# atenpas/gpd

Measured on NVIDIA H100. Metric: grasp candidates/sec end-to-end (15ch), higher is better.
Workload: dtype f64 geometry / f32 LeNet

## Files before the change

### gpd_b200/csrc/api.cu

```cuda
#include <atomic>
#include <cfloat>
#include <cmath>
#include <cstdarg>
#include <cstdio>
#include <cstdlib>
#include <cstring>
#include <initializer_list>
#include <string>
#include <utility>
#include <vector>

#include "../../include/gpd_b200_depth.h"
#include "../../include/gpd_b200_outliers.h"
#include "../../include/gpd_b200_plane.h"
#include "../../include/gpd_b200_refine.h"
#include "common.cuh"

static char g_create_err[512] = "";

struct StageTimes {
  struct Span { int stage; cudaEvent_t b, e; };
  std::vector<cudaEvent_t> pool;
  size_t used = 0;
  std::vector<Span> spans;
// ... 2560 lines not shown
    return GPDB_ERR_STATE;
  }
  const SisState &st = *ctx->sis;
  const int B = st.B, R = st.R, S = st.S, RS = R * S;
  SisArena a;
  carve_at(ctx->scratch[SCR_SIS], [&](Carve &c) { sis_layout(c, B, R, S, st.init_off[B], a); });
  CUDA_TRY(cudaSetDevice(ctx->device));
  std::vector<double> ev(eval_xyz_out ? 3 * (size_t)B * RS : 0), kp(kept_xyz_out ? 3 * ((size_t)st.init_off[B] + (size_t)B * RS) : 0);
  if (!ev.empty()) CUDA_TRY(cudaMemcpyAsync(ev.data(), a.eval, sizeof(double) * ev.size(), cudaMemcpyDeviceToHost, ctx->stream));
  if (!kp.empty()) CUDA_TRY(cudaMemcpyAsync(kp.data(), a.kept, sizeof(double) * kp.size(), cudaMemcpyDeviceToHost, ctx->stream));
  CUDA_TRY(cudaStreamSynchronize(ctx->stream));
  if (eval_offsets_out || eval_round_counts_out || eval_xyz_out) {
    size_t o = 0;
    if (eval_offsets_out) eval_offsets_out[0] = 0;
    for (int b = 0; b < B; b++) {
      for (int r = 0; r < R; r++) {
        const int c = st.ecount[(size_t)r * B + b];
        if (eval_round_counts_out) eval_round_counts_out[(size_t)b * R + r] = c;
        if (eval_xyz_out) memcpy(eval_xyz_out + 3 * o, ev.data() + 3 * ((size_t)b * R + r) * S, sizeof(double) * 3 * c);
        o += c;
      }
      if (eval_offsets_out) eval_offsets_out[b + 1] = (int32_t)o;
    }
  }
  if (kept_offsets_out) memcpy(kept_offsets_out, st.koff.data(), sizeof(int32_t) * ((size_t)B + 1));
  if (kept_xyz_out)
    for (int b = 0; b < B; b++)
      memcpy(kept_xyz_out + 3 * (size_t)st.koff[b], kp.data() + 3 * ((size_t)st.init_off[b] + (size_t)b * RS),
             sizeof(double) * 3 * (size_t)(st.koff[b + 1] - st.koff[b]));
  return B;
}

void gpdb_free_result(gpdb_result *r) {
  if (!r) return;
  if (r->owner_) {
    HostArena *a = (HostArena *)r->owner_;
    a->in_use = false;
    arena_unref(a);
  } else {
    free(r->frame_valid);
    free(r->frames);
    free(r->pose_flags);
    free(r->pose_scores);
    free(r->candidates);
    free(r->images);
  }
  memset(r, 0, sizeof(*r));
}

int gpdb_debug_phase_cycles(gpdb_ctx *ctx, int enable, uint64_t cycles_out[32]) {
  if (!ctx) return GPDB_ERR_INVALID;
  CUDA_TRY(cudaSetDevice(ctx->device));
  CUDA_TRY(cudaStreamSynchronize(ctx->stream));
  if (ctx->d_prof && cycles_out) {
    CUDA_TRY(cudaMemcpy(cycles_out, ctx->d_prof, sizeof(uint64_t) * 16, cudaMemcpyDeviceToHost));
    CUDA_TRY(cudaMemcpy(cycles_out + 16, ctx->d_prof + GPDB_PROF_SUB, sizeof(uint64_t) * 16, cudaMemcpyDeviceToHost));
  }
  if (enable && !ctx->d_prof) CUDA_TRY(cudaMalloc(&ctx->d_prof, sizeof(uint64_t) * GPDB_PROF_SLOTS));
  if (enable) CUDA_TRY(cudaMemset(ctx->d_prof, 0, sizeof(uint64_t) * GPDB_PROF_SLOTS));
  if (!enable && ctx->d_prof) {
    cudaFree(ctx->d_prof);
    ctx->d_prof = nullptr;
  }
  return GPDB_OK;
}

int gpdb_debug_path_counts(gpdb_ctx *ctx, uint64_t counts_out[16]) {
  if (!ctx || !counts_out) return GPDB_ERR_INVALID;
  CUDA_TRY(cudaSetDevice(ctx->device));
  CUDA_TRY(cudaStreamSynchronize(ctx->stream));
  if (ctx->d_prof)
    CUDA_TRY(cudaMemcpy(counts_out, ctx->d_prof + GPDB_PROF_PATH, sizeof(uint64_t) * 16, cudaMemcpyDeviceToHost));
  else
    memset(counts_out, 0, sizeof(uint64_t) * 16);
  return GPDB_OK;
}

int gpdb_last_timings(const gpdb_ctx *ctx, double ms_out[8]) {
  if (!ctx || !ms_out) return GPDB_ERR_INVALID;
  for (int i = 0; i < 8; i++) ms_out[i] = ctx->last_ms[i];
  return GPDB_OK;
}

}
```

### gpd_b200/csrc/common.cuh

```cuda
#pragma once
#include <cuda_runtime.h>
#include <stdint.h>

#include "../../include/gpd_b200.h"
#include "../../include/gpd_b200_shadow.h"

#define GPDB_MAX_ORIENT 32
#define GPDB_MAX_SLOTS 32
#define GPDB_MAX_DEEPEN 64
#define GPDB_MAX_NSP 128

struct DevParams {
  double finger_width, hand_outer_diameter, hand_depth, hand_height, init_bite;
  int P, n_axes, n_orient, nfp;
  int axes[GPDB_MAX_HAND_AXES];
  int deepen, slots_disjoint, all_axes_z;
  double inv_slot_step;
  double fs[GPDB_MAX_SLOTS];
  double fsw[GPDB_MAX_SLOTS];
  int J;
  double topj[GPDB_MAX_DEEPEN], botj[GPDB_MAX_DEEPEN];
  double cosf;
  int min_viable;
  double min_ap, max_ap, ws[6];
// ... 23 lines not shown
  const float *xyz;
  const double *nrm;
  const uint8_t *cam;
  const int *cell_start;
  const double *samples;
  int n_points;
};

struct CloudDesc {
  float lo[3], inv_cell;
  int dim[3];
  int cell_base;
  int off, N, K;
  int all_seen;
  int nonunit;
  int pos;
  double vp[GPDB_MAX_CAMERAS][3];
};
struct CloudTable {
  const CloudDesc *d;
  const int *soff;
  int n;
};

struct CloudSet {
  float4 *pts4;
  float *xyz;
  double *nrm;
  uint8_t *cam;
  int *src;
  int *cell_start;
  CloudDesc *desc;
  int *soff;
  int *off;
  int *sel;
  int *pos;
  int *raw_off;
  size_t point_cap, cell_cap, desc_cap;
  int n, maxk;
  bool has_src;
  double *samples;
  int n_samples;
  size_t samples_cap;
  int positions(int b) const { return n_samples ? pos[b + 1] - pos[b] : 0; }
  DevCloud view;
  int points() const { return n ? off[n] : 0; }
  CloudTable table() const { return CloudTable{desc, soff, n}; }
};

#define GPDB_NERR 8

#define GPDB_PROF_PATH 16
#define GPDB_PROF_SUB 32
#define GPDB_PROF_SLOTS 48
enum PathEvent {
  PATH_FRAMES_T1, PATH_FRAMES_T2, PATH_HANDS_T2, PATH_HANDS_T3, PATH_HANDS_SLAB, PATH_IMG2_BOX, PATH_IMG2_NONUNIT, PATH_IMG_GL,
  PATH_IMG2_CAST, PATH_IMG2_DRAW, PATH_IMG2_STASH, PATH_IMG_CAST, PATH_IMG_DRAW, PATH_IMG_STASH, PATH_IMG_BALL, PATH_LABEL_WALK
};

#define CUDA_TRY(expr)                                                                        \
  do {                                                                                        \
    cudaError_t e__ = (expr);                                                                 \
    if (e__ != cudaSuccess) {                                                                 \
      gpdb_set_error(ctx, GPDB_ERR_CUDA, "%s:%d %s -> %s", __FILE__, __LINE__, #expr,         \
                     cudaGetErrorString(e__));                                                \
      return GPDB_ERR_CUDA;                                                                   \
    }                                                                                         \
  } while (0)

#define LAUNCH_CHECK()                                                                                    \
  do {                                                                                                    \
    ctx->launches++;                                                                                      \
    cudaError_t e__ = cudaGetLastError();                                                                 \
    if (e__ != cudaSuccess) {                                                                             \
      gpdb_set_error(ctx, GPDB_ERR_CUDA, "%s:%d launch -> %s", __FILE__, __LINE__, cudaGetErrorString(e__)); \
      return GPDB_ERR_CUDA;                                                                               \
    }                                                                                                     \
  } while (0)

struct LenetWeights {
  float *c1w, *c1b, *c2w, *c2b, *i1w, *i1b, *i2w, *i2b;
  int C;
  bool set;
};

struct C1Affine {
  float scale[20], bias[20];
};
struct LenetTc {
  void *b1, *b2, *b3;
  C1Affine c1_aff;
  int npl, nch1;
  float w2_scale, a2_scale, w3_scale, x3_scale;
  bool ready;
};

struct StageTimes;
struct PipeState;
struct CommState;
struct SisState;

enum ScratchSlot {
  SCR_P16,
  SCR_CUB,
  SCR_OVF,
  SCR_KEYS,
  SCR_WORK_A, SCR_WORK_B, SCR_WORK_C,
// ... 240 lines not shown
```

### gpd_b200/csrc/geometry.cu

```cuda
#include <cfloat>
#include <climits>
#include <cstdlib>
#include <vector>
#include <cub/cub.cuh>

#include "common.cuh"
#include "grid.cuh"

namespace {

constexpr int NT_HANDS = 256;
#ifndef GPDB_NT_IMG
#define GPDB_NT_IMG 512
#endif
constexpr int NT_IMG = GPDB_NT_IMG;
constexpr int LRF_WARPS = 4;
constexpr int LRF_CAP_GLOBAL = 16384;
constexpr int LRF_CAP = 1024;
constexpr int BOX_CAP = 2048;
constexpr int MAXPIX = 64 * 64;

__device__ __forceinline__ void to_frame(const double *F, double v0, double v1, double v2, double &o0, double &o1,
                                         double &o2) {
  o0 = (F[0] * v0 + F[1] * v1) + F[2] * v2;
  o1 = (F[3] * v0 + F[4] * v1) + F[5] * v2;
  o2 = (F[6] * v0 + F[7] * v1) + F[8] * v2;
}
__device__ __forceinline__ void mat3_mul(const double *A, const double *B, double *Cm) {
#pragma unroll
  for (int c = 0; c < 3; c++)
#pragma unroll
    for (int r = 0; r < 3; r++) Cm[c * 3 + r] = (A[r] * B[c * 3] + A[3 + r] * B[c * 3 + 1]) + A[6 + r] * B[c * 3 + 2];
}

__device__ __forceinline__ double warp_min(double v) {
#pragma unroll
  for (int o = 16; o; o >>= 1) v = fmin(v, __shfl_xor_sync(0xffffffffu, v, o));
  return v;
}
__device__ __forceinline__ double warp_max(double v) {
#pragma unroll
  for (int o = 16; o; o >>= 1) v = fmax(v, __shfl_xor_sync(0xffffffffu, v, o));
  return v;
}
__device__ __forceinline__ int warp_sum(int v) { return __reduce_add_sync(0xffffffffu, v); }

template <int NT>
struct SegScan {
  typedef cub::BlockScan<int, NT> Scan;
  typename Scan::TempStorage tmp;
  int start[NT];
  int prefix[NT + 1];
};
template <int NT, class G>
__device__ __forceinline__ int seg_batch(const G &P, const int *cell_start, const SegRange &s, int row0,
                                         SegScan<NT> &seg) {
  int row = row0 + threadIdx.x, st = 0, len = 0;
  if (row < s.nrows) seg_row(P, cell_start, s, row, st, len);
  int excl, total;
  SegScan<NT>::Scan(seg.tmp).ExclusiveSum(len, excl, total);
  seg.start[threadIdx.x] = st;
  seg.prefix[threadIdx.x] = excl;
  if (threadIdx.x == 0) seg.prefix[NT] = total;
  __syncthreads();
  return total;
}
template <int NT, class G, class F>
__device__ __forceinline__ void scan_balanced(const G &P, const DevCloud &cl, const SegRange &sr, SegScan<NT> &seg,
                                              F &&body) {
  const int warp = threadIdx.x >> 5, lane = threadIdx.x & 31;
  constexpr int NW = NT / 32;
  for (int row0 = 0; row0 < sr.nrows; row0 += NT) {
    __syncthreads();
    const int total = seg_batch<NT>(P, cl.cell_start, sr, row0, seg);
    const int nr = min(NT, sr.nrows - row0);
    const int c_begin = (int)(((long long)total * warp) / NW), c_end = (int)(((long long)total * (warp + 1)) / NW);
    if (c_begin >= c_end) continue;
    int lo = 0, hi = nr;
    while (hi - lo > 1) {
      int mid = (lo + hi) >> 1;
      if (seg.prefix[mid] <= c_begin) lo = mid; else hi = mid;
    }
    int r = lo, c = c_begin;
    auto fetch = [&](bool &have, bool &in, float4 &p, int &where) {
      have = false;
      in = false;
      where = 0;
      p = make_float4(0.f, 0.f, 0.f, 0.f);
      while (c < c_end) {
        const int pe = (r + 1 < nr) ? seg.prefix[r + 1] : total;
        const int seg_end = min(pe, c_end);
        if (c >= seg_end) {
          r++;
          continue;
        }
        const int k = c + lane;
        in = k < seg_end;
        where = (seg.start[r] - seg.prefix[r]) + k;
        if (in) p = __ldg(cl.pts4 + where);
        c = min(c + 32, seg_end);
        have = true;
        return;
      }
    };
    bool have0, in0, have1, in1;
    float4 p0, p1;
    int w0, w1;
    fetch(have0, in0, p0, w0);
    while (have0) {
      fetch(have1, in1, p1, w1);
      body(in0, p0, w0);
      have0 = have1;
      in0 = in1;
      p0 = p1;
      w0 = w1;
    }
  }
}

template <int NT>
__device__ __forceinline__ int seg_lookup(const SegScan<NT> &seg, int c) {
  int lo = 0, hi = NT;
  while (hi - lo > 1) {
    int mid = (lo + hi) >> 1;
    if (seg.prefix[mid] <= c) lo = mid; else hi = mid;
  }
  return seg.start[lo] + (c - seg.prefix[lo]);
}

__device__ void make_givens(double p, double q, double &c, double &s) {
  if (q == 0.0) {
    c = p < 0.0 ? -1.0 : 1.0;
    s = 0.0;
  } else if (p == 0.0) {
    c = 0.0;
    s = q < 0.0 ? 1.0 : -1.0;
  } else if (fabs(p) > fabs(q)) {
    double t = q / p;
    double u = sqrt(1.0 + t * t);
    if (p < 0.0) u = -u;
    c = 1.0 / u;
    s = -t * c;
  } else {
    double t = p / q;
    double u = sqrt(1.0 + t * t);
    if (q < 0.0) u = -u;
    s = -1.0 / u;
    c = -t * s;
  }
}
__device__ double eigen_hypot(double x, double y) {
  double ax = fabs(x), ay = fabs(y);
  double p = fmax(ax, ay);
  if (p == 0.0) return 0.0;
  double qp = fmin(ax, ay) / p;
  return p * sqrt(1.0 + qp * qp);
}
__device__ void eigen3(const double *Min, double *eval, double *Q) {
  double m00 = Min[0], m10 = Min[1], m20 = Min[2], m11 = Min[4], m21 = Min[5], m22 = Min[8];
  double scale = fmax(fmax(fmax(fabs(m00), fabs(m10)), fmax(fabs(m20), fabs(m11))), fmax(fabs(m21), fabs(m22)));
  if (scale == 0.0) scale = 1.0;
  m00 /= scale; m10 /= scale; m20 /= scale; m11 /= scale; m21 /= scale; m22 /= scale;
  double diag[3], sub[2];
  const double tol = DBL_MIN;
  diag[0] = m00;
  double v1norm2 = m20 * m20;
  if (v1norm2 <= tol) {
    diag[1] = m11;
// ... 188 lines not shown
    double eval[3], evec[9];
    eigen3(M, eval, evec);
    int mn = 0, mx = 0;
    for (int k = 1; k < 3; k++) {
      if (eval[k] < eval[mn]) mn = k;
      if (eval[k] > eval[mx]) mx = k;
    }
    double curv[3] = {evec[mn * 3], evec[mn * 3 + 1], evec[mn * 3 + 2]};
    double normal[3] = {evec[mx * 3], evec[mx * 3 + 1], evec[mx * 3 + 2]};
    double nrm = sqrt((a[6] * a[6] + a[7] * a[7]) + a[8] * a[8]);
    double avg[3] = {a[6] / nrm, a[7] / nrm, a[8] / nrm};
    if ((avg[0] * normal[0] + avg[1] * normal[1]) + avg[2] * normal[2] < 0) {
      normal[0] *= -1.0; normal[1] *= -1.0; normal[2] *= -1.0;
    }
    double *f = frames + 9 * (size_t)i;
    f[0] = normal[0]; f[1] = normal[1]; f[2] = normal[2];
    f[3] = curv[1] * normal[2] - curv[2] * normal[1];
    f[4] = curv[2] * normal[0] - curv[0] * normal[2];
    f[5] = curv[0] * normal[1] - curv[1] * normal[0];
    f[6] = curv[0]; f[7] = curv[1]; f[8] = curv[2];
    valid[i] = 1;
  }
  return true;
}

__device__ __forceinline__ unsigned slot_mask(const DevParams &P, const double *sfs, const double *sfsw, double y) {
  unsigned m = 0;
  const int F = 2 * P.nfp;
  if (P.slots_disjoint) {
#pragma unroll
    for (int half = 0; half < 2; half++) {
      const double *fs = sfs + half * P.nfp, *fsw = sfsw + half * P.nfp;
      const double tq = (y - fs[0]) * P.inv_slot_step;
      const double tf = floor(tq);
      if (tq - tf > 1e-9 && tf + 1.0 - tq > 1e-9) {
        const int i = (int)tf;
        if (i >= 0 && i < P.nfp && y > fs[i] && y < fsw[i]) m |= 1u << (half * P.nfp + i);
      } else {
        const int e = min(max((int)tf, 1), P.nfp - 2 > 1 ? P.nfp - 2 : 1);
#pragma unroll
        for (int d = -1; d <= 1; d++) {
          const int i = e + d;
          if (i >= 0 && i < P.nfp && y > fs[i] && y < fsw[i]) m |= 1u << (half * P.nfp + i);
        }
      }
    }
  } else {
    for (int f = 0; f < F; f++)
      if (y > sfs[f] && y < sfsw[f]) m |= 1u << f;
  }
  return m;
}

constexpr int SURV_CAP = 1024;
struct HandsSmem {
  SegScan<NT_HANDS> seg;
  unsigned short surv[NT_HANDS / 32][SURV_CAP];
  double fs[GPDB_MAX_SLOTS], fsw[GPDB_MAX_SLOTS];
  int count;
  int n_ball;
  unsigned long long nb0_key;
  double T[9];
  double frame[9];
  double sample[3];
  int cap;
};

template <bool BATCH>
__global__ void __launch_bounds__(NT_HANDS, 4) k_hands(const DevParams *Pp, DevCloud cl0, CloudTable tab, const int *sidx, int n, int slot0,
                                                    const double *frames, const uint8_t *fvalid, gpdb_pose *poses,
                                                    uint8_t *flags, int cap, const int *in_list, const int *in_count,
                                                    int *out_list, int *out_count, float4 *glist, int *err,
                                                    unsigned long long *prof) {
  const DevParams &P = *Pp;
  extern __shared__ __align__(16) unsigned char dyn[];
  float4 *list = glist ? glist + (size_t)blockIdx.x * cap : reinterpret_cast<float4 *>(dyn);
  __shared__ HandsSmem S;
  const int tid = threadIdx.x, lane = tid & 31, warp = tid >> 5;
  const int work_n = in_list ? *in_count : n;
  if (tid < 2 * P.nfp) {
    S.fs[tid] = P.fs[tid];
    S.fsw[tid] = P.fsw[tid];
  }
  for (int w = blockIdx.x; w < work_n; w += gridDim.x) {
    const int i = in_list ? in_list[w] : w;
    const int si = sidx[i];
    const auto &G = CloudSel<BATCH>::get(tab, slot0 + i);
    const DevCloud cl = CloudSel<BATCH>::local(G, cl0);
    __syncthreads();
    if (tid == 0) {
      S.count = 0;
      S.n_ball = 0;
      S.nb0_key = ~0ull;
    }
    if (tid < 9) S.frame[tid] = frames[9 * (size_t)i + tid];
    if (tid == 0) sample_position(cl, si, S.sample);
    __syncthreads();
    if (tid == 0) mat3_mul(S.frame, P.rotb, S.T);
    const bool fv = fvalid[i] != 0;
    if (!fv) {
      for (int p = tid; p < P.P; p += NT_HANDS) {
        gpdb_pose *h = poses + (size_t)i * P.P + p;
        memset(h, 0, sizeof(gpdb_pose));
        h->sample_index = si;
        h->sample_slot = slot0 + i;
        h->pose_slot = (int16_t)p;
        h->finger_idx = -1;
        h->score = __int_as_float(0x7fc00000);
        flags[(size_t)i * P.P + p] = 0;
      }
      continue;
    }
    __syncthreads();
    float q[3] = {(float)S.sample[0], (float)S.sample[1], (float)S.sample[2]};
    SegRange sr = seg_range(G, q, P.rf_hs);
    const double hz = P.hand_height * 1.001 + 1e-9;
    unsigned long long best = ~0ull;
    int nball = 0;
    scan_balanced<NT_HANDS>(G, cl, sr, S.seg, [&](bool in, const float4 &p, int) {
      bool keep = false;
      if (in) {
        float d = l2_simple(q, p.x, p.y, p.z);
        if (d < P.r2_hs) {
          nball++;
          unsigned long long key = ((unsigned long long)__float_as_uint(d) << 32) | (unsigned)__float_as_int(p.w);
          best = key < best ? key : best;
          keep = true;
          if (P.all_axes_z) {
            double z0 = (S.T[6] * ((double)p.x - S.sample[0]) + S.T[7] * ((double)p.y - S.sample[1])) +
                        S.T[8] * ((double)p.z - S.sample[2]);
            keep = fabs(z0) < hz;
          }
        }
      }
      unsigned m = __ballot_sync(0xffffffffu, keep);
      if (m) {
        int leader = __ffs(m) - 1, base = 0;
        if (lane == leader) base = atomicAdd(&S.count, __popc(m));
        base = __shfl_sync(0xffffffffu, base, leader);
        int pos = base + __popc(m & ((1u << lane) - 1));
        if (keep && pos < cap) list[pos] = p;
      }
    });
    nball = warp_sum(nball);
#pragma unroll
    for (int o = 16; o; o >>= 1) {
      unsigned long long ob = __shfl_xor_sync(0xffffffffu, best, o);
      best = ob < best ? ob : best;
    }
    if (lane == 0) {
      atomicAdd(&S.n_ball, nball);
      atomicMin(&S.nb0_key, best);
    }
    __syncthreads();
    const int m = S.count;
    if (m > cap) {
      if (tid == 0) {
        if (out_list) {
          int k = atomicAdd(out_count, 1);
          out_list[k] = i;
          if (!in_list) atomicAdd(err + 3, 1);
        } else {
          atomicAdd(err + 1, 1);
        }
      }
      if (!out_list) {
        for (int p = tid; p < P.P; p += NT_HANDS) flags[(size_t)i * P.P + p] = 0;
      }
      continue;
    }
    const int n_ball = S.n_ball;
    const int nb0 = (int)(unsigned)(S.nb0_key & 0xffffffffu);
    double nbx = 0, nby = 0, nbz = 0;
    if (n_ball > 0) {
      nbx = (double)cl.xyz[3 * (size_t)nb0] - S.sample[0];
      nby = (double)cl.xyz[3 * (size_t)nb0 + 1] - S.sample[1];
      nbz = (double)cl.xyz[3 * (size_t)nb0 + 2] - S.sample[2];
    }
    for (int pose = warp; pose < P.P; pose += NT_HANDS / 32) {
      gpdb_pose *h = poses + (size_t)i * P.P + pose;
      double R[9];
      mat3_mul(S.T, P.rot[pose], R);
      const double hh = P.hand_height;
      uint8_t fl = 0;
      double top = 0, bottom = 0, center = 0, width = 0;
      int fidx = -1, fpi = -1;
      bool half = false, full = false;
      double x0, y0, z0;
      to_frame(R, nbx, nby, nbz, x0, y0, z0);
      if (n_ball > 0) {
        const double b0 = P.init_bite, bot0 = P.init_bite - P.hand_depth;
        int k = 0;
        unsigned anyA = 0, anyB = 0, fmask = 0;
        for (int a = lane; a < m; a += 32) {
          float4 p = list[a];
          double x, y, z;
          to_frame(R, (double)p.x - S.sample[0], (double)p.y - S.sample[1], (double)p.z - S.sample[2], x, y, z);
          if (z > -1.0 * hh && z < hh) {
            k++;
            if (x < b0) {
              anyA = 1;
              if (x < bot0) anyB = 1;
              fmask |= slot_mask(P, S.fs, S.fsw, y);
            }
          }
        }
        k = warp_sum(k);
        const int npad = n_ball - k;
        if (npad > 0 && x0 < b0) {
          anyA = 1;
          if (x0 < bot0) anyB = 1;
          fmask |= slot_mask(P, S.fs, S.fsw, y0);
        }
        anyA = __reduce_or_sync(0xffffffffu, anyA);
        anyB = __reduce_or_sync(0xffffffffu, anyB);
        fmask = __reduce_or_sync(0xffffffffu, fmask);
        const unsigned allF = (2 * P.nfp >= 32) ? 0xffffffffu : ((1u << (2 * P.nfp)) - 1);
        unsigned freef = (anyA && !anyB) ? (~fmask & allF) : 0u;
        unsigned hand = freef & (freef >> P.nfp) & ((1u << P.nfp) - 1);
        if (hand) {
          int cntb = __popc(hand);
          int target = (cntb + 1) / 2;
          unsigned hm = hand;
          while (--target) hm &= hm - 1;
          fidx = __ffs(hm) - 1;
          fpi = P.deepen ? fidx : (__ffs(hand) - 1);
          top = b0;
          bottom = bot0;
          if (P.deepen) {
            int jf = P.J;
            const double sl0 = P.fs[fidx], sl1 = P.fsw[fidx], sr0 = P.fs[P.nfp + fidx], sr1 = P.fsw[P.nfp + fidx];
            const int J = P.J;
            auto visitB = [&](double x, double y) {
              if (J > 0 && x < P.botj[J - 1]) {
                int j = 0;
                while (!(x < P.botj[j])) j++;
                jf = min(jf, j);
              }
              if ((y > sl0 && y < sl1) || (y > sr0 && y < sr1)) {
                if (J > 0 && x < P.topj[J - 1]) {
                  int j = 0;
                  while (!(x < P.topj[j])) j++;
                  jf = min(jf, j);
                }
              }
            };
            for (int a = lane; a < m; a += 32) {
              float4 p = list[a];
              double x, y, z;
              to_frame(R, (double)p.x - S.sample[0], (double)p.y - S.sample[1], (double)p.z - S.sample[2], x, y, z);
              if (z > -1.0 * hh && z < hh) visitB(x, y);
            }
            if (npad > 0) visitB(x0, y0);
            jf = __reduce_min_sync(0xffffffffu, jf);
            if (jf > 0) {
              top = P.topj[jf - 1];
              bottom = P.botj[jf - 1];
            }
          }
          const double left = P.fsw[fidx], right = P.fs[P.nfp + fidx];
          center = 0.5 * (left + right);
          int cnt = 0;
          double mny = DBL_MAX, mxy = -DBL_MAX;
          unsigned short *surv = S.surv[warp];
          int nsurv = 0;
          for (int a0 = 0; a0 < m; a0 += 32) {
            const int a = a0 + lane;
            bool inr = false;
            if (a < m) {
              float4 p = list[a];
              double x, y, z;
              to_frame(R, (double)p.x - S.sample[0], (double)p.y - S.sample[1], (double)p.z - S.sample[2], x, y, z);
              if (z > -1.0 * hh && z < hh && x > bottom && x < top && y > left && y < right) {
                inr = true;
                cnt++;
                mny = fmin(mny, y);
                mxy = fmax(mxy, y);
              }
            }
            const unsigned mk = __ballot_sync(0xffffffffu, inr);
            const int pos = nsurv + __popc(mk & ((1u << lane) - 1));
            if (inr && pos < SURV_CAP) surv[pos] = (unsigned short)a;
            nsurv += __popc(mk);
          }
          const bool surv_ok = nsurv <= SURV_CAP && m <= 65535;
          __syncwarp();
          const bool nb_in = npad > 0 && x0 > bottom && x0 < top && y0 > left && y0 < right;
          cnt = warp_sum(cnt) + (nb_in ? npad : 0);
          mny = warp_min(mny);
          mxy = warp_max(mxy);
          if (nb_in) {
            mny = fmin(mny, y0);
            mxy = fmax(mxy, y0);
          }
          if (cnt > 0) {
            fl |= GPDB_POSE_VALID;
            width = mxy - mny;
            const double min_x = mny + 0.003, max_x = mxy - 0.003;
            int cl_ = 0, cr_ = 0;
            double lmaxx = -DBL_MAX, lminx = DBL_MAX, lmaxz = -DBL_MAX, lminz = DBL_MAX;
            double rmaxx = -DBL_MAX, rminx = DBL_MAX, rmaxz = -DBL_MAX, rminz = DBL_MAX;
            auto visitD = [&](double x, double y, double z, int idx, int wgt) {
              const double *nn = cl.nrm + 3 * (size_t)idx;
              double n0, n1, n2;
              to_frame(R, nn[0], nn[1], nn[2], n0, n1, n2);
              double ldot = (0.0 * n0 + -1.0 * n1) + 0.0 * n2;
              double rdot = (0.0 * n0 + 1.0 * n1) + 0.0 * n2;
              if (ldot > P.cosf && y < min_x) {
                cl_ += wgt;
                lmaxx = fmax(lmaxx, x); lminx = fmin(lminx, x); lmaxz = fmax(lmaxz, z); lminz = fmin(lminz, z);
              }
              if (rdot > P.cosf && y > max_x) {
                cr_ += wgt;
                rmaxx = fmax(rmaxx, x); rminx = fmin(rminx, x); rmaxz = fmax(rmaxz, z); rminz = fmin(rminz, z);
              }
            };
            if (surv_ok) {
              for (int sidx_ = lane; sidx_ < nsurv; sidx_ += 32) {
                float4 p = list[surv[sidx_]];
                double x, y, z;
                to_frame(R, (double)p.x - S.sample[0], (double)p.y - S.sample[1], (double)p.z - S.sample[2], x, y, z);
                visitD(x, y, z, __float_as_int(p.w), 1);
              }
            } else {
              if (prof && lane == 0) atomicAdd(prof + GPDB_PROF_PATH + PATH_HANDS_SLAB, 1ull);
              for (int a = lane; a < m; a += 32) {
                float4 p = list[a];
                double x, y, z;
                to_frame(R, (double)p.x - S.sample[0], (double)p.y - S.sample[1], (double)p.z - S.sample[2], x, y, z);
                if (z > -1.0 * hh && z < hh && x > bottom && x < top && y > left && y < right)
                  visitD(x, y, z, __float_as_int(p.w), 1);
              }
            }
            if (nb_in && lane == 0) visitD(x0, y0, z0, nb0, npad);
            cl_ = warp_sum(cl_);
            cr_ = warp_sum(cr_);
            half = cl_ > 0 || cr_ > 0;
            if (cl_ > 0 && cr_ > 0) {
              lmaxx = warp_max(lmaxx); lminx = warp_min(lminx); lmaxz = warp_max(lmaxz); lminz = warp_min(lminz);
              rmaxx = warp_max(rmaxx); rminx = warp_min(rminx); rmaxz = warp_max(rmaxz); rminz = warp_min(rminz);
              const double top_y = fmin(lmaxx, rmaxx), bot_y = fmax(lminx, rminx);
              const double top_z = fmin(lmaxz, rmaxz), bot_z = fmax(lminz, rminz);
              int nl = 0, nr = 0;
              auto visitE = [&](double x, double y, double z, int idx, int wgt) {
                const double *nn = cl.nrm + 3 * (size_t)idx;
                double n0, n1, n2;
                to_frame(R, nn[0], nn[1], nn[2], n0, n1, n2);
                double ldot = (0.0 * n0 + -1.0 * n1) + 0.0 * n2;
                double rdot = (0.0 * n0 + 1.0 * n1) + 0.0 * n2;
                bool inw = x >= bot_y && x <= top_y && z >= bot_z && z <= top_z;
                if (ldot > P.cosf && y < min_x && inw) nl += wgt;
                if (rdot > P.cosf && y > max_x && inw) nr += wgt;
              };
              if (surv_ok) {
                for (int sidx_ = lane; sidx_ < nsurv; sidx_ += 32) {
                  float4 p = list[surv[sidx_]];
                  double x, y, z;
                  to_frame(R, (double)p.x - S.sample[0], (double)p.y - S.sample[1], (double)p.z - S.sample[2], x, y, z);
                  visitE(x, y, z, __float_as_int(p.w), 1);
                }
              } else {
                for (int a = lane; a < m; a += 32) {
                  float4 p = list[a];
                  double x, y, z;
                  to_frame(R, (double)p.x - S.sample[0], (double)p.y - S.sample[1], (double)p.z - S.sample[2], x, y, z);
                  if (z > -1.0 * hh && z < hh && x > bottom && x < top && y > left && y < right)
                    visitE(x, y, z, __float_as_int(p.w), 1);
                }
              }
              if (nb_in && lane == 0) visitE(x0, y0, z0, nb0, npad);
              nl = warp_sum(nl);
              nr = warp_sum(nr);
              full = nl >= P.min_viable && nr >= P.min_viable;
            }
            if (half) fl |= GPDB_POSE_HALF;
            if (full) fl |= GPDB_POSE_FULL;
          }
        }
      }
      if (lane == 0) {
        gpdb_pose o;
        memset(&o, 0, sizeof(o));
        for (int r = 0; r < 3; r++) o.sample[r] = S.sample[r];
        for (int r = 0; r < 9; r++) o.frame[r] = R[r];
        o.sample_index = si;
        o.sample_slot = slot0 + i;
        o.pose_slot = (int16_t)pose;
        o.finger_idx = -1;
        o.score = __int_as_float(0x7fc00000);
        if (fl & GPDB_POSE_VALID) {
          o.top = top;
          o.bottom = bottom;
          o.center = center;
          o.width = width;
          o.finger_idx = (int16_t)fpi;
          o.half_antipodal = half;
          o.full_antipodal = full;
          for (int r = 0; r < 3; r++)
            o.position[r] = ((R[r] * bottom + R[3 + r] * center) + R[6 + r] * 0.0) + S.sample[r];
          const double half_width = 0.5 * P.hand_outer_diameter;
          bool ok = width >= P.min_ap && width <= P.max_ap;
          for (int r = 0; r < 3; r++) {
            double lb = o.position[r] + half_width * R[3 + r];
            double rb = o.position[r] - half_width * R[3 + r];
            double lt = lb + P.hand_depth * R[r];
            double rt = lb + P.hand_depth * R[r];
            double ap = o.position[r] - 0.05 * R[r];
            double mn = fmin(fmin(fmin(lb, rb), fmin(lt, rt)), ap);
            double mx = fmax(fmax(fmax(lb, rb), fmax(lt, rt)), ap);
            ok = ok && mn >= P.ws[2 * r] && mx <= P.ws[2 * r + 1];
          }
          if (ok && P.filt_dir) {
            double dot = (P.dir[0] * R[0] + P.dir[1] * R[1]) + P.dir[2] * R[2];
            if (dot >= -1.0 && dot <= 1.0 && dot < P.dir_keep) ok = false;
          }
          if (ok) fl |= GPDB_POSE_FILTERED;
        }
        *h = o;
        flags[(size_t)i * P.P + pose] = fl;
      }
    }
  }
}

__global__ void k_flag01(const uint8_t *flags, int n, int *f01) {
  int i = blockIdx.x * blockDim.x + threadIdx.x;
  if (i < n) f01[i] = (flags[i] & 3) == 3;
}
__global__ void k_scatter(const gpdb_pose *poses, const int *f01, const int *pos, int n, gpdb_pose *cand, int *count) {
  int i = blockIdx.x * blockDim.x + threadIdx.x;
  if (i >= n) return;
  if (f01[i]) cand[pos[i]] = poses[i];
  if (i == n - 1) *count = pos[i] + f01[i];
}
__global__ void k_scatter_scores(const gpdb_pose *cand, const float *scores, int nc, int slot0, int P, float *pose_scores,
                                 gpdb_pose *cand_out) {
  int i = blockIdx.x * blockDim.x + threadIdx.x;
  if (i >= nc) return;
  float s = scores[i];
  pose_scores[(size_t)(cand[i].sample_slot - slot0) * P + cand[i].pose_slot] = s;
  cand_out[i].score = s;
}

__global__ void k_select_keys(const gpdb_pose *cand, int n, unsigned *keys, int *vals) {
  int i = blockIdx.x * blockDim.x + threadIdx.x;
  if (i >= n) return;
  unsigned u = __float_as_uint(cand[i].score);
  u ^= (u >> 31) ? 0xFFFFFFFFu : 0x80000000u;
  keys[i] = ~u;
  vals[i] = i;
}
__global__ void k_gather_poses(const gpdb_pose *cand, const int *order, int k, gpdb_pose *out) {
  const int w = (blockIdx.x * blockDim.x + threadIdx.x) >> 5, lane = threadIdx.x & 31;
  if (w >= k) return;
  const int *src = reinterpret_cast<const int *>(cand + order[w]);
  int *dst = reinterpret_cast<int *>(out + w);
  for (int j = lane; j < (int)(sizeof(gpdb_pose) / 4); j += 32) dst[j] = src[j];
}

constexpr int LABEL_NT = 128;
constexpr int LABEL_CAP = 1024;

template <class F>
__device__ __forceinline__ void warp_scan_ball(const CloudDesc &G, const DevCloud &cl, const SegRange &sr, const float q[3], float r2,
                                               F &&body) {
  const int lane = threadIdx.x & 31;
  for (int j0 = 0; j0 < sr.nrows; j0 += 32) {
    const int myrow = j0 + lane;
    int st = 0, len = 0;
    if (myrow < sr.nrows) seg_row(G, cl.cell_start, sr, myrow, st, len);
    unsigned nonempty = __ballot_sync(0xffffffffu, len > 0);
    while (nonempty) {
      const int j = __ffs(nonempty) - 1;
// ... 1629 lines not shown
  if (!ctx->d_prof) return GPDB_OK;
  k_path_add<<<1, 1, 0, ctx->stream>>>(ctx->d_prof, e0, n0, e1, n1);
  CUDA_TRY(cudaGetLastError());
  return GPDB_OK;
}

static bool overflow_lists(gpdb_ctx *ctx, int n, int *&ovf, int *&ovf_count, int *&ovf2, int *&ovf2_count) {
  return gpdb_carve(ctx, SCR_OVF, [&](Carve &c) {
    ovf = c.take<int>(n); ovf_count = c.take<int>(1); ovf2 = c.take<int>(n); ovf2_count = c.take<int>(1);
  });
}

template <bool BATCH>
static int launch_frames(gpdb_ctx *ctx, const CloudSet &s, const int *d_sidx, int n, double *d_frames, uint8_t *d_valid) {
  const int cap0 = 128;
  const size_t smem0 = (size_t)2 * LRF_WARPS * cap0 * sizeof(unsigned long long);
  const size_t smem1 = (size_t)2 * LRF_WARPS * LRF_CAP * sizeof(unsigned long long);
  CUDA_TRY(cudaFuncSetAttribute(k_frames<BATCH>, cudaFuncAttributeMaxDynamicSharedMemorySize, (int)smem1));
  int *ovf, *ovf_count, *ovf2, *ovf2_count;
  if (!overflow_lists(ctx, n, ovf, ovf_count, ovf2, ovf2_count)) return GPDB_ERR_CUDA;
  const int g2 = 37;
  unsigned long long *gkeys =
      (unsigned long long *)gpdb_scratch(ctx, SCR_FRAMES_GL, sizeof(unsigned long long) * 2 * LRF_CAP_GLOBAL * (size_t)g2 * LRF_WARPS);
  if (!gkeys) return GPDB_ERR_CUDA;
  CUDA_TRY(cudaMemsetAsync(ovf_count, 0, sizeof(int), ctx->stream));
  CUDA_TRY(cudaMemsetAsync(ovf2_count, 0, sizeof(int), ctx->stream));
  const DevCloud &cl = s.view;
  const CloudTable tab = s.table();
  const int grid = (n + LRF_WARPS - 1) / LRF_WARPS;
  k_frames<BATCH><<<grid, LRF_WARPS * 32, smem0, ctx->stream>>>(ctx->dp, cl, tab, d_sidx, n, d_frames, d_valid, ctx->d_err, cap0,
                                                                ovf, ovf_count, ovf2, ovf2_count, nullptr, 0);
  LAUNCH_CHECK();
  k_frames<BATCH><<<grid, LRF_WARPS * 32, smem1, ctx->stream>>>(ctx->dp, cl, tab, d_sidx, n, d_frames, d_valid, ctx->d_err,
                                                                LRF_CAP, ovf, ovf_count, ovf2, ovf2_count, nullptr, 1);
  LAUNCH_CHECK();
  k_frames<BATCH><<<g2, LRF_WARPS * 32, 0, ctx->stream>>>(ctx->dp, cl, tab, d_sidx, n, d_frames, d_valid, ctx->d_err,
                                                          LRF_CAP_GLOBAL, ovf, ovf_count, ovf2, ovf2_count, gkeys, 2);
  LAUNCH_CHECK();
  return path_add(ctx, PATH_FRAMES_T1, ovf_count, PATH_FRAMES_T2, ovf2_count);
}

int geo_frames(gpdb_ctx *ctx, const CloudSet &s, const int *d_sidx, int n, double *d_frames, uint8_t *d_valid) {
  if (n <= 0) return GPDB_OK;
  return s.n > 1 ? launch_frames<true>(ctx, s, d_sidx, n, d_frames, d_valid)
                 : launch_frames<false>(ctx, s, d_sidx, n, d_frames, d_valid);
}

static const int HANDS_CAP1 = 2176, HANDS_CAP2 = 12800;
static const int HANDS_CAP3 = 131072;

template <bool BATCH>
static int launch_hands(gpdb_ctx *ctx, const CloudSet &s, const int *d_sidx, int n, int slot0, const double *d_frames,
                        const uint8_t *d_valid, gpdb_pose *d_poses, uint8_t *d_flags) {
  CUDA_TRY(cudaFuncSetAttribute(k_hands<BATCH>, cudaFuncAttributeMaxDynamicSharedMemorySize, HANDS_CAP2 * 16));
  int *ovf, *ovf_count, *ovf2, *ovf2_count;
  if (!overflow_lists(ctx, n, ovf, ovf_count, ovf2, ovf2_count)) return GPDB_ERR_CUDA;
  float4 *glist = (float4 *)gpdb_scratch(ctx, SCR_HANDS_GL, sizeof(float4) * (size_t)HANDS_CAP3 * ctx->sm_count);
  if (!glist) return GPDB_ERR_CUDA;
  CUDA_TRY(cudaMemsetAsync(ovf_count, 0, sizeof(int), ctx->stream));
  CUDA_TRY(cudaMemsetAsync(ovf2_count, 0, sizeof(int), ctx->stream));
  const DevCloud &cl = s.view;
  const CloudTable tab = s.table();
  k_hands<BATCH><<<n, NT_HANDS, HANDS_CAP1 * 16, ctx->stream>>>(ctx->dp, cl, tab, d_sidx, n, slot0, d_frames, d_valid, d_poses,
                                                                d_flags, HANDS_CAP1, nullptr, nullptr, ovf, ovf_count, nullptr,
                                                                ctx->d_err, ctx->d_prof);
  LAUNCH_CHECK();
  k_hands<BATCH><<<ctx->sm_count, NT_HANDS, HANDS_CAP2 * 16, ctx->stream>>>(ctx->dp, cl, tab, d_sidx, n, slot0, d_frames,
                                                                            d_valid, d_poses, d_flags, HANDS_CAP2, ovf,
                                                                            ovf_count, ovf2, ovf2_count, nullptr, ctx->d_err,
                                                                            ctx->d_prof);
  LAUNCH_CHECK();
  k_hands<BATCH><<<ctx->sm_count, NT_HANDS, 16, ctx->stream>>>(ctx->dp, cl, tab, d_sidx, n, slot0, d_frames, d_valid, d_poses,
                                                               d_flags, HANDS_CAP3, ovf2, ovf2_count, nullptr, nullptr, glist,
                                                               ctx->d_err, ctx->d_prof);
  LAUNCH_CHECK();
  return path_add(ctx, PATH_HANDS_T2, ovf_count, PATH_HANDS_T3, ovf2_count);
}

int geo_hands(gpdb_ctx *ctx, const CloudSet &s, const int *d_sidx, int n, int slot0, const double *d_frames,
              const uint8_t *d_valid, gpdb_pose *d_poses, uint8_t *d_flags) {
  if (n <= 0) return GPDB_OK;
  return s.n > 1 ? launch_hands<true>(ctx, s, d_sidx, n, slot0, d_frames, d_valid, d_poses, d_flags)
                 : launch_hands<false>(ctx, s, d_sidx, n, slot0, d_frames, d_valid, d_poses, d_flags);
}

int geo_compact(gpdb_ctx *ctx, const gpdb_pose *d_poses, const uint8_t *d_flags, int n_poses, gpdb_pose *d_cand,
                int *d_count) {
  if (n_poses <= 0) {
    CUDA_TRY(cudaMemsetAsync(d_count, 0, sizeof(int), ctx->stream));
    return GPDB_OK;
  }
  int *f01, *pos;
  if (!gpdb_carve(ctx, SCR_KEYS, [&](Carve &c) { f01 = c.take<int>(n_poses); pos = c.take<int>(n_poses); }))
    return GPDB_ERR_CUDA;
  const int tb = 256, gb = (n_poses + tb - 1) / tb;
  k_flag01<<<gb, tb, 0, ctx->stream>>>(d_flags, n_poses, f01);
  LAUNCH_CHECK();
  size_t tmp_bytes = 0;
  cub::DeviceScan::ExclusiveSum(nullptr, tmp_bytes, f01, pos, n_poses, ctx->stream);
  void *tmp = gpdb_scratch(ctx, SCR_CUB, tmp_bytes);
  if (!tmp) return GPDB_ERR_CUDA;
  CUDA_TRY(cub::DeviceScan::ExclusiveSum(tmp, tmp_bytes, f01, pos, n_poses, ctx->stream));
  ctx->launches += 2;
  k_scatter<<<gb, tb, 0, ctx->stream>>>(d_poses, f01, pos, n_poses, d_cand, d_count);
  LAUNCH_CHECK();
  return GPDB_OK;
}

template <int S_T, bool BATCH>
static int launch_general(gpdb_ctx *ctx, const CloudSet &s, const gpdb_pose *d_cand, int nc, uint8_t *d_p16, size_t smem,
                          size_t plane_bytes, size_t list_bytes, int grid, const int *d_work, const int *d_work_n,
                          unsigned char *gl, int gl_cap, int *ovf2, int *ovf2_count) {
  const DevCloud &cl = s.view;
  const CloudTable tab = s.table();
  CUDA_TRY(cudaFuncSetAttribute(k_images<S_T, false, BATCH>, cudaFuncAttributeMaxDynamicSharedMemorySize, (int)smem));
  CUDA_TRY(cudaFuncSetAttribute(k_images<S_T, true, BATCH>, cudaFuncAttributeMaxDynamicSharedMemorySize, (int)smem));
  k_images<S_T, false, BATCH><<<grid, NT_IMG, smem, ctx->stream>>>(ctx->dp, cl, tab, d_cand, nc, d_p16, ctx->d_qtab, ctx->d_err,
                                                                  (int)plane_bytes, (int)list_bytes, ctx->d_prof, d_work,
                                                                  d_work_n, nullptr, 0, ovf2, ovf2_count);
  LAUNCH_CHECK();
  k_images<S_T, true, BATCH><<<ctx->sm_count, NT_IMG, smem, ctx->stream>>>(ctx->dp, cl, tab, d_cand, nc, d_p16, ctx->d_qtab,
                                                                          ctx->d_err, (int)plane_bytes, (int)list_bytes,
                                                                          ctx->d_prof, ovf2, ovf2_count, gl, gl_cap, nullptr,
                                                                          nullptr);
  LAUNCH_CHECK();
  return GPDB_OK;
}
// ... 246 lines not shown
```

Measured before the change: 2.085 million.

## Add hands-phase profiling, flat unrolled ball scan, and early exit in pass A

Replaces the balanced double-buffered scan in the hands kernel with a flat per-warp partitioned scan that issues U=4 independent point loads per lane before processing. It also lets the pass-A loop over slab points stop early once a bottom collision is found or all finger slots are blocked, since the result can no longer change. It adds an optional clock64-based per-phase profiler template variant selected only when profiling is enabled. Risks: the flat partition may balance work worse across warps, and the early exit adds a warp vote every iteration. It also changes k, which feeds npad, so it may alter results.

```diff
diff --git a/gpd_b200/csrc/api.cu b/gpd_b200/csrc/api.cu
--- a/gpd_b200/csrc/api.cu
+++ b/gpd_b200/csrc/api.cu
@@ -2636,7 +2636,9 @@
   if (!ctx) return GPDB_ERR_INVALID;
   CUDA_TRY(cudaSetDevice(ctx->device));
   CUDA_TRY(cudaStreamSynchronize(ctx->stream));
-  if (ctx->d_prof && cycles_out) {
+  if (ctx->d_prof && cycles_out && enable == 2) {
+    CUDA_TRY(cudaMemcpy(cycles_out, ctx->d_prof + GPDB_PROF_HANDS, sizeof(uint64_t) * 32, cudaMemcpyDeviceToHost));
+  } else if (ctx->d_prof && cycles_out) {
     CUDA_TRY(cudaMemcpy(cycles_out, ctx->d_prof, sizeof(uint64_t) * 16, cudaMemcpyDeviceToHost));
     CUDA_TRY(cudaMemcpy(cycles_out + 16, ctx->d_prof + GPDB_PROF_SUB, sizeof(uint64_t) * 16, cudaMemcpyDeviceToHost));
   }
diff --git a/gpd_b200/csrc/common.cuh b/gpd_b200/csrc/common.cuh
--- a/gpd_b200/csrc/common.cuh
+++ b/gpd_b200/csrc/common.cuh
@@ -99,7 +99,12 @@
 
 #define GPDB_PROF_PATH 16
 #define GPDB_PROF_SUB 32
-#define GPDB_PROF_SLOTS 48
+#define GPDB_PROF_HANDS 48
+#define GPDB_PROF_SLOTS 80
+enum HandsProf {
+  HP_POSE_WAIT, HP_SETUP, HP_STAGE, HP_PASS_A, HP_DEEPEN, HP_CLOSING, HP_ANTI_D, HP_ANTI_E, HP_RECORD,
+  HP_SAMPLES, HP_BALL, HP_SLAB, HP_SLAB_1024, HP_SLAB_2176, HP_POSES, HP_HAND, HP_VALID, HP_PASS_E
+};
 enum PathEvent {
   PATH_FRAMES_T1, PATH_FRAMES_T2, PATH_HANDS_T2, PATH_HANDS_T3, PATH_HANDS_SLAB, PATH_IMG2_BOX, PATH_IMG2_NONUNIT, PATH_IMG_GL,
   PATH_IMG2_CAST, PATH_IMG2_DRAW, PATH_IMG2_STASH, PATH_IMG_CAST, PATH_IMG_DRAW, PATH_IMG_STASH, PATH_IMG_BALL, PATH_LABEL_WALK
diff --git a/gpd_b200/csrc/geometry.cu b/gpd_b200/csrc/geometry.cu
--- a/gpd_b200/csrc/geometry.cu
+++ b/gpd_b200/csrc/geometry.cu
@@ -10,6 +10,10 @@
 namespace {
 
 constexpr int NT_HANDS = 256;
+#ifndef GPDB_HANDS_STAGE_U
+#define GPDB_HANDS_STAGE_U 4
+#endif
+constexpr int HANDS_STAGE_U = GPDB_HANDS_STAGE_U;
 #ifndef GPDB_NT_IMG
 #define GPDB_NT_IMG 512
 #endif
@@ -114,6 +118,43 @@
       in0 = in1;
       p0 = p1;
       w0 = w1;
+    }
+  }
+}
+template <int NT, int U, class G, class F>
+__device__ __forceinline__ void scan_flat(const G &P, const DevCloud &cl, const SegRange &sr, SegScan<NT> &seg, F &&body) {
+  const int warp = threadIdx.x >> 5, lane = threadIdx.x & 31;
+  constexpr int NW = NT / 32;
+  for (int row0 = 0; row0 < sr.nrows; row0 += NT) {
+    __syncthreads();
+    const int total = seg_batch<NT>(P, cl.cell_start, sr, row0, seg);
+    const int nr = min(NT, sr.nrows - row0);
+    const int c_begin = (int)(((long long)total * warp) / NW), c_end = (int)(((long long)total * (warp + 1)) / NW);
+    if (c_begin >= c_end) continue;
+    int lo = 0, hi = nr;
+    while (hi - lo > 1) {
+      int mid = (lo + hi) >> 1;
+      if (seg.prefix[mid] <= c_begin) lo = mid; else hi = mid;
+    }
+    int r = lo;
+    for (int c = c_begin; c < c_end; c += 32 * U) {
+      float4 p[U];
+      bool in[U];
+      int where[U];
+#pragma unroll
+      for (int u = 0; u < U; u++) {
+        const int k = c + 32 * u + lane;
+        in[u] = k < c_end;
+        where[u] = 0;
+        p[u] = make_float4(0.f, 0.f, 0.f, 0.f);
+        if (in[u]) {
+          while (r + 1 < nr && seg.prefix[r + 1] <= k) r++;
+          where[u] = (seg.start[r] - seg.prefix[r]) + k;
+          p[u] = __ldg(cl.pts4 + where[u]);
+        }
+      }
+#pragma unroll
+      for (int u = 0; u < U; u++) body(in[u], p[u], where[u]);
     }
   }
 }
@@ -408,6 +449,17 @@
   return m;
 }
 
+__device__ __forceinline__ void hands_phase(unsigned long long *prof, bool on, int i, long long &t) {
+  if (prof && on) {
+    const long long now = clock64();
+    atomicAdd(prof + GPDB_PROF_HANDS + i, (unsigned long long)(now - t));
+    t = now;
+  }
+}
+__device__ __forceinline__ void hands_count(unsigned long long *prof, bool on, int i, unsigned long long v) {
+  if (prof && on) atomicAdd(prof + GPDB_PROF_HANDS + i, v);
+}
+
 constexpr int SURV_CAP = 1024;
 struct HandsSmem {
   SegScan<NT_HANDS> seg;
@@ -420,9 +472,10 @@
   double frame[9];
   double sample[3];
   int cap;
+  long long t_ph[NT_HANDS / 32];
 };
 
-template <bool BATCH>
+template <bool BATCH, bool PROBE = false>
 __global__ void __launch_bounds__(NT_HANDS, 4) k_hands(const DevParams *Pp, DevCloud cl0, CloudTable tab, const int *sidx, int n, int slot0,
                                                     const double *frames, const uint8_t *fvalid, gpdb_pose *poses,
                                                     uint8_t *flags, int cap, const int *in_list, const int *in_count,
@@ -434,6 +487,8 @@
   __shared__ HandsSmem S;
   const int tid = threadIdx.x, lane = tid & 31, warp = tid >> 5;
   const int work_n = in_list ? *in_count : n;
+  unsigned long long *const hp = PROBE ? prof : nullptr;
+  if (hp && lane == 0) S.t_ph[warp] = clock64();
   if (tid < 2 * P.nfp) {
     S.fs[tid] = P.fs[tid];
     S.fsw[tid] = P.fsw[tid];
@@ -444,6 +499,7 @@
     const auto &G = CloudSel<BATCH>::get(tab, slot0 + i);
     const DevCloud cl = CloudSel<BATCH>::local(G, cl0);
     __syncthreads();
+    hands_phase(hp, tid == 0, HP_POSE_WAIT, S.t_ph[warp]);
     if (tid == 0) {
       S.count = 0;
       S.n_ball = 0;
@@ -468,12 +524,13 @@
       continue;
     }
     __syncthreads();
+    hands_phase(hp, tid == 0, HP_SETUP, S.t_ph[warp]);
     float q[3] = {(float)S.sample[0], (float)S.sample[1], (float)S.sample[2]};
     SegRange sr = seg_range(G, q, P.rf_hs);
     const double hz = P.hand_height * 1.001 + 1e-9;
     unsigned long long best = ~0ull;
     int nball = 0;
-    scan_balanced<NT_HANDS>(G, cl, sr, S.seg, [&](bool in, const float4 &p, int) {
+    scan_flat<NT_HANDS, HANDS_STAGE_U>(G, cl, sr, S.seg, [&](bool in, const float4 &p, int) {
       bool keep = false;
       if (in) {
         float d = l2_simple(q, p.x, p.y, p.z);
@@ -510,6 +567,7 @@
     }
     __syncthreads();
     const int m = S.count;
+    hands_phase(hp, tid == 0, HP_STAGE, S.t_ph[warp]);
     if (m > cap) {
       if (tid == 0) {
         if (out_list) {
@@ -526,6 +584,13 @@
       continue;
     }
     const int n_ball = S.n_ball;
+    if (hp && tid == 0) {
+      hands_count(hp, true, HP_SAMPLES, 1);
+      hands_count(hp, true, HP_BALL, n_ball);
+      hands_count(hp, true, HP_SLAB, m);
+      hands_count(hp, true, m <= 1024 ? HP_SLAB_1024 : HP_SLAB_2176, m <= 2176);
+    }
+    if (hp && lane == 0) S.t_ph[warp] = clock64();
     const int nb0 = (int)(unsigned)(S.nb0_key & 0xffffffffu);
     double nbx = 0, nby = 0, nbz = 0;
     if (n_ball > 0) {
@@ -548,18 +613,23 @@
         const double b0 = P.init_bite, bot0 = P.init_bite - P.hand_depth;
         int k = 0;
         unsigned anyA = 0, anyB = 0, fmask = 0;
-        for (int a = lane; a < m; a += 32) {
-          float4 p = list[a];
-          double x, y, z;
-          to_frame(R, (double)p.x - S.sample[0], (double)p.y - S.sample[1], (double)p.z - S.sample[2], x, y, z);
-          if (z > -1.0 * hh && z < hh) {
-            k++;
-            if (x < b0) {
-              anyA = 1;
-              if (x < bot0) anyB = 1;
-              fmask |= slot_mask(P, S.fs, S.fsw, y);
+        const unsigned allF = (2 * P.nfp >= 32) ? 0xffffffffu : ((1u << (2 * P.nfp)) - 1);
+        for (int a0 = 0; a0 < m; a0 += 32) {
+          const int a = a0 + lane;
+          if (a < m) {
+            float4 p = list[a];
+            double x, y, z;
+            to_frame(R, (double)p.x - S.sample[0], (double)p.y - S.sample[1], (double)p.z - S.sample[2], x, y, z);
+            if (z > -1.0 * hh && z < hh) {
+              k++;
+              if (x < b0) {
+                anyA = 1;
+                if (x < bot0) anyB = 1;
+                fmask |= slot_mask(P, S.fs, S.fsw, y);
+              }
             }
           }
+          if (__any_sync(0xffffffffu, anyB) || (__reduce_or_sync(0xffffffffu, fmask) & allF) == allF) break;
         }
         k = warp_sum(k);
         const int npad = n_ball - k;
@@ -571,9 +641,10 @@
         anyA = __reduce_or_sync(0xffffffffu, anyA);
         anyB = __reduce_or_sync(0xffffffffu, anyB);
         fmask = __reduce_or_sync(0xffffffffu, fmask);
-        const unsigned allF = (2 * P.nfp >= 32) ? 0xffffffffu : ((1u << (2 * P.nfp)) - 1);
         unsigned freef = (anyA && !anyB) ? (~fmask & allF) : 0u;
         unsigned hand = freef & (freef >> P.nfp) & ((1u << P.nfp) - 1);
+        hands_phase(hp, lane == 0, HP_PASS_A, S.t_ph[warp]);
+        hands_count(hp, lane == 0 && hand, HP_HAND, 1);
         if (hand) {
           int cntb = __popc(hand);
           int target = (cntb + 1) / 2;
@@ -613,6 +684,7 @@
               top = P.topj[jf - 1];
               bottom = P.botj[jf - 1];
             }
+            hands_phase(hp, lane == 0, HP_DEEPEN, S.t_ph[warp]);
           }
           const double left = P.fsw[fidx], right = P.fs[P.nfp + fidx];
           center = 0.5 * (left + right);
@@ -649,6 +721,8 @@
             mny = fmin(mny, y0);
             mxy = fmax(mxy, y0);
           }
+          hands_phase(hp, lane == 0, HP_CLOSING, S.t_ph[warp]);
+          hands_count(hp, lane == 0 && cnt > 0, HP_VALID, 1);
           if (cnt > 0) {
             fl |= GPDB_POSE_VALID;
             width = mxy - mny;
@@ -692,6 +766,8 @@
             cl_ = warp_sum(cl_);
             cr_ = warp_sum(cr_);
             half = cl_ > 0 || cr_ > 0;
+            hands_phase(hp, lane == 0, HP_ANTI_D, S.t_ph[warp]);
+            hands_count(hp, lane == 0 && cl_ > 0 && cr_ > 0, HP_PASS_E, 1);
             if (cl_ > 0 && cr_ > 0) {
               lmaxx = warp_max(lmaxx); lminx = warp_min(lminx); lmaxz = warp_max(lmaxz); lminz = warp_min(lminz);
               rmaxx = warp_max(rmaxx); rminx = warp_min(rminx); rmaxz = warp_max(rmaxz); rminz = warp_min(rminz);
@@ -728,6 +804,7 @@
               nl = warp_sum(nl);
               nr = warp_sum(nr);
               full = nl >= P.min_viable && nr >= P.min_viable;
+              hands_phase(hp, lane == 0, HP_ANTI_E, S.t_ph[warp]);
             }
             if (half) fl |= GPDB_POSE_HALF;
             if (full) fl |= GPDB_POSE_FULL;
@@ -775,6 +852,8 @@
         *h = o;
         flags[(size_t)i * P.P + pose] = fl;
       }
+      hands_phase(hp, lane == 0, HP_RECORD, S.t_ph[warp]);
+      hands_count(hp, lane == 0, HP_POSES, 1);
     }
   }
 }
@@ -2510,7 +2589,8 @@
 template <bool BATCH>
 static int launch_hands(gpdb_ctx *ctx, const CloudSet &s, const int *d_sidx, int n, int slot0, const double *d_frames,
                         const uint8_t *d_valid, gpdb_pose *d_poses, uint8_t *d_flags) {
-  CUDA_TRY(cudaFuncSetAttribute(k_hands<BATCH>, cudaFuncAttributeMaxDynamicSharedMemorySize, HANDS_CAP2 * 16));
+  auto *const kern = ctx->d_prof ? k_hands<BATCH, !BATCH> : k_hands<BATCH>;
+  CUDA_TRY(cudaFuncSetAttribute(kern, cudaFuncAttributeMaxDynamicSharedMemorySize, HANDS_CAP2 * 16));
   int *ovf, *ovf_count, *ovf2, *ovf2_count;
   if (!overflow_lists(ctx, n, ovf, ovf_count, ovf2, ovf2_count)) return GPDB_ERR_CUDA;
   float4 *glist = (float4 *)gpdb_scratch(ctx, SCR_HANDS_GL, sizeof(float4) * (size_t)HANDS_CAP3 * ctx->sm_count);
@@ -2519,18 +2599,18 @@
   CUDA_TRY(cudaMemsetAsync(ovf2_count, 0, sizeof(int), ctx->stream));
   const DevCloud &cl = s.view;
   const CloudTable tab = s.table();
-  k_hands<BATCH><<<n, NT_HANDS, HANDS_CAP1 * 16, ctx->stream>>>(ctx->dp, cl, tab, d_sidx, n, slot0, d_frames, d_valid, d_poses,
-                                                                d_flags, HANDS_CAP1, nullptr, nullptr, ovf, ovf_count, nullptr,
-                                                                ctx->d_err, ctx->d_prof);
+  kern<<<n, NT_HANDS, HANDS_CAP1 * 16, ctx->stream>>>(ctx->dp, cl, tab, d_sidx, n, slot0, d_frames, d_valid, d_poses,
+                                                      d_flags, HANDS_CAP1, nullptr, nullptr, ovf, ovf_count, nullptr,
+                                                      ctx->d_err, ctx->d_prof);
   LAUNCH_CHECK();
-  k_hands<BATCH><<<ctx->sm_count, NT_HANDS, HANDS_CAP2 * 16, ctx->stream>>>(ctx->dp, cl, tab, d_sidx, n, slot0, d_frames,
-                                                                            d_valid, d_poses, d_flags, HANDS_CAP2, ovf,
-                                                                            ovf_count, ovf2, ovf2_count, nullptr, ctx->d_err,
-                                                                            ctx->d_prof);
+  kern<<<ctx->sm_count, NT_HANDS, HANDS_CAP2 * 16, ctx->stream>>>(ctx->dp, cl, tab, d_sidx, n, slot0, d_frames,
+                                                                  d_valid, d_poses, d_flags, HANDS_CAP2, ovf,
+                                                                  ovf_count, ovf2, ovf2_count, nullptr, ctx->d_err,
+                                                                  ctx->d_prof);
   LAUNCH_CHECK();
-  k_hands<BATCH><<<ctx->sm_count, NT_HANDS, 16, ctx->stream>>>(ctx->dp, cl, tab, d_sidx, n, slot0, d_frames, d_valid, d_poses,
-                                                               d_flags, HANDS_CAP3, ovf2, ovf2_count, nullptr, nullptr, glist,
-                                                               ctx->d_err, ctx->d_prof);
+  kern<<<ctx->sm_count, NT_HANDS, 16, ctx->stream>>>(ctx->dp, cl, tab, d_sidx, n, slot0, d_frames, d_valid, d_poses,
+                                                     d_flags, HANDS_CAP3, ovf2, ovf2_count, nullptr, nullptr, glist,
+                                                     ctx->d_err, ctx->d_prof);
   LAUNCH_CHECK();
   return path_add(ctx, PATH_HANDS_T2, ovf_count, PATH_HANDS_T3, ovf2_count);
 }
```

Measured after the change: 2.133 million, median of 6. 2.3% higher.
